# achiever04/face-recognition-platform

Hardware: AMD Instinct MI355X
Metric: faces/sec (detect+embed+match) on 1080p @ 100k gallery (higher is better)
Workload: dtype f16; 1 GPU; 32x1080x1920 BGR frames per GPU per step resident in HBM, host results out every step, 2 batches in flight per GPU (one handle = one stream each, used round-robin), forced K=10 faces/frame, 100000-identity fp16 gallery, FRPDet detector fp16 + ArcFace IResNet-100 fp16 (synthetic seeded weights); batch_frames=32, faces_per_frame=10, gallery=100000, streams=1, lanes=2, lane_warmup_steps=20

## Files before the change

face-recognition-platform_amd/csrc/aux_kernels.hip:

```cpp
#include <hip/hip_runtime.h>
#include <stdint.h>
#include "frp_internal.h"

namespace frp {

typedef _Float16 half8 __attribute__((ext_vector_type(8)));

__global__ __launch_bounds__(256) void preprocess_kernel(const uint8_t* __restrict__ src, int B, int H, int W,
                                                         long row_stride, long frame_stride,
                                                         _Float16* __restrict__ out, int Hc, int Wc, int rgb_in) {
    const long total = (long)B * Hc * Wc;
    for (long i = (long)blockIdx.x * blockDim.x + threadIdx.x; i < total; i += (long)gridDim.x * blockDim.x) {
        const int x = (int)(i % Wc);
        const long r = i / Wc;
        const int y = (int)(r % Hc);
        const int b = (int)(r / Hc);
        float c0 = 0.f, c1 = 0.f, c2 = 0.f;
        if (y < H && x < W) {
            const uint8_t* p = src + b * frame_stride + y * row_stride + 3L * x;
            c0 = (float)p[0]; c1 = (float)p[1]; c2 = (float)p[2];
        }
        const float r_ = rgb_in ? c0 : c2, g_ = c1, b_ = rgb_in ? c2 : c0;
        half8 v;
        v[0] = (_Float16)((r_ - 127.5f) * (1.0f / 128.0f));
// ... 11 lines not shown
    const int grid = (int)((total + 255) / 256 < 16384 ? (total + 255) / 256 : 16384);
    hipLaunchKernelGGL(preprocess_kernel, dim3(grid), dim3(256), 0, stream, bgr, B, H, W, row_stride, frame_stride,
                       out, Hc, Wc, rgb_in);
    return hipGetLastError();
}

__global__ __launch_bounds__(256) void compact_faces_kernel(const int32_t* __restrict__ counts, int B, int max_faces,
                                                            int32_t* __restrict__ face_slot, int32_t* __restrict__ n_faces) {
    __shared__ int offs[1024 + 1];
    if (threadIdx.x == 0) {
        int acc = 0;
        for (int b = 0; b < B; ++b) { offs[b] = acc; acc += counts[b]; }
        offs[B] = acc;
        *n_faces = acc;
    }
    __syncthreads();
    for (int b = threadIdx.x; b < B; b += blockDim.x) {
        const int c = counts[b], o = offs[b];
        for (int k = 0; k < c; ++k) face_slot[o + k] = b * max_faces + k;
    }
}

hipError_t launch_compact_faces(const int32_t* counts, int B, int max_faces, int32_t* face_slot, int32_t* n_faces,
                                hipStream_t stream) {
    if (B <= 0 || B > 1024) return hipErrorInvalidValue;
    hipLaunchKernelGGL(compact_faces_kernel, dim3(1), dim3(256), 0, stream, counts, B, max_faces, face_slot, n_faces);
    return hipGetLastError();
}

__constant__ float kTemplate[10] = {38.2946f, 51.6963f, 73.5318f, 51.5014f, 56.0252f, 71.7366f,
                                    41.5493f, 92.3655f, 70.7299f, 92.2041f};

#define ALIGN_SPLIT 7
__global__ __launch_bounds__(256) void align_kernel(AlignParams p) {
    const int f = blockIdx.x / ALIGN_SPLIT, part = blockIdx.x - f * ALIGN_SPLIT;
    if (f >= p.n_faces || (p.n_dev && f >= *p.n_dev)) return;
    const int slot = p.face_slot ? p.face_slot[f] : f;
    const int b = p.face_slot ? slot / p.max_faces : 0;
    const float* k = p.kps + (long)slot * 10;
    double msx = 0, msy = 0, mdx = 0, mdy = 0;
    for (int i = 0; i < 5; ++i) { msx += k[2 * i]; msy += k[2 * i + 1]; mdx += kTemplate[2 * i]; mdy += kTemplate[2 * i + 1]; }
    msx /= 5; msy /= 5; mdx /= 5; mdy /= 5;
    double num_a = 0, num_b = 0, den = 0;
    for (int i = 0; i < 5; ++i) {
        const double sx = k[2 * i] - msx, sy = k[2 * i + 1] - msy;
        const double dx = kTemplate[2 * i] - mdx, dy = kTemplate[2 * i + 1] - mdy;
        num_a += sx * dx + sy * dy;
        num_b += sx * dy - sy * dx;
        den += sx * sx + sy * sy;
    }
    const bool ok = den > 1e-12 && (num_a * num_a + num_b * num_b) > 1e-24;
    const double a = ok ? num_a / den : 1.0, bb = ok ? num_b / den : 0.0;
    const double tx = mdx - (a * msx - bb * msy), ty = mdy - (bb * msx + a * msy);
    const double det = a * a + bb * bb;
    const float i00 = (float)(a / det), i01 = (float)(bb / det), i10 = (float)(-bb / det), i11 = (float)(a / det);
    const float itx = (float)(-(a * tx + bb * ty) / det), ity = (float)(-(-bb * tx + a * ty) / det);
    const uint8_t* img = p.frames + (long)b * p.frame_stride;
    _Float16* out = p.chips + (long)f * (FRP_CHIP_PIX * 8);
    const int c_r = p.rgb_in ? 0 : 2, c_b = p.rgb_in ? 2 : 0;
    constexpr int kPart = FRP_CHIP_PIX / ALIGN_SPLIT;
    static_assert(kPart * ALIGN_SPLIT == FRP_CHIP_PIX, "chip rows must split evenly");
    for (int i = part * kPart + threadIdx.x; i < (part + 1) * kPart; i += blockDim.x) {
        const int v = i / 112, u = i - v * 112;
        const float sx = fminf(fmaxf(i00 * (float)u + i01 * (float)v + itx, -2.f), (float)(p.W + 1));
        const float sy = fminf(fmaxf(i10 * (float)u + i11 * (float)v + ity, -2.f), (float)(p.H + 1));
        const float fx0 = floorf(sx), fy0 = floorf(sy);
        const int x0 = (int)fx0, y0 = (int)fy0;
        const float ax = sx - fx0, ay = sy - fy0;
        unsigned char tap[4][3];
        float wgt[4];
        const int bx_max = 3 * p.W - 8;
        int bx = 3 * x0;
        bx = bx < 0 ? 0 : (bx > bx_max ? bx_max : bx);
#pragma unroll
        for (int dy = 0; dy < 2; ++dy) {
            const int yy = y0 + dy;
            const int yc = yy < 0 ? 0 : (yy >= p.H ? p.H - 1 : yy);
            unsigned long long v;
            __builtin_memcpy(&v, img + (long)yc * p.row_stride + bx, 8);
#pragma unroll
            for (int dx = 0; dx < 2; ++dx) {
                const int xx = x0 + dx;
                const bool inside = ok && (unsigned)xx < (unsigned)p.W && (unsigned)yy < (unsigned)p.H;
                int o = 3 * xx - bx;
                o = o < 0 ? 0 : (o > 5 ? 5 : o);
                const unsigned pix = (unsigned)(v >> (8 * o));
                tap[dy * 2 + dx][0] = (unsigned char)(pix >> (8 * c_r));
                tap[dy * 2 + dx][1] = (unsigned char)(pix >> 8);
                tap[dy * 2 + dx][2] = (unsigned char)(pix >> (8 * c_b));
                wgt[dy * 2 + dx] = inside ? (dx ? ax : 1.f - ax) * (dy ? ay : 1.f - ay) : 0.f;
            }
        }
        float acc[3] = {0.f, 0.f, 0.f};
#pragma unroll
        for (int k = 0; k < 4; ++k) {
            acc[0] += wgt[k] * (float)tap[k][0];
            acc[1] += wgt[k] * (float)tap[k][1];
            acc[2] += wgt[k] * (float)tap[k][2];
        }
        half8 o;
        o[0] = (_Float16)((acc[0] - 127.5f) * (1.0f / 127.5f));
        o[1] = (_Float16)((acc[1] - 127.5f) * (1.0f / 127.5f));
        o[2] = (_Float16)((acc[2] - 127.5f) * (1.0f / 127.5f));
        o[3] = o[4] = o[5] = o[6] = o[7] = (_Float16)0.f;
        *reinterpret_cast<half8*>(out + (long)i * 8) = o;
    }
}

hipError_t launch_align(const AlignParams& p, hipStream_t stream) {
    if (p.n_faces <= 0) return hipSuccess;
    if (!p.frames || !p.kps || !p.chips || p.H <= 0 || p.W < 3) return hipErrorInvalidValue;
    hipLaunchKernelGGL(align_kernel, dim3(p.n_faces * ALIGN_SPLIT), dim3(256), 0, stream, p);
    return hipGetLastError();
}

__global__ __launch_bounds__(256) void chips_to_blob_kernel(const uint8_t* __restrict__ chips, long total,
                                                            _Float16* __restrict__ out) {
    for (long i = (long)blockIdx.x * blockDim.x + threadIdx.x; i < total; i += (long)gridDim.x * blockDim.x) {
        const uint8_t* p = chips + 3 * i;
        half8 o;
        o[0] = (_Float16)(((float)p[2] - 127.5f) * (1.0f / 127.5f));
        o[1] = (_Float16)(((float)p[1] - 127.5f) * (1.0f / 127.5f));
        o[2] = (_Float16)(((float)p[0] - 127.5f) * (1.0f / 127.5f));
        o[3] = o[4] = o[5] = o[6] = o[7] = (_Float16)0.f;
        *reinterpret_cast<half8*>(out + i * 8) = o;
    }
}

hipError_t launch_chips_to_blob(const uint8_t* chips, int M, _Float16* out, hipStream_t stream) {
    if (M <= 0) return hipSuccess;
    const long total = (long)M * FRP_CHIP_PIX;
    const int grid = (int)((total + 255) / 256 < 8192 ? (total + 255) / 256 : 8192);
    hipLaunchKernelGGL(chips_to_blob_kernel, dim3(grid), dim3(256), 0, stream, chips, total, out);
    return hipGetLastError();
}

__device__ __forceinline__ float wave_sum(float v) {
#pragma unroll
    for (int o = 32; o > 0; o >>= 1) v += __shfl_xor(v, o);
    return v;
}

__global__ __launch_bounds__(256) void l2norm_kernel(float* __restrict__ emb, _Float16* __restrict__ emb16, int M, int D,
                                                      const float* __restrict__ partials, int ksplit, const float* __restrict__ bias,
                                                      const int32_t* __restrict__ n_dev, int fc_ktot, int n_cu) {
// ... 181 lines not shown
```

face-recognition-platform_amd/csrc/decode_nms.hip:

```cpp
#include <hip/hip_runtime.h>
#include <stdint.h>
#include "frp_internal.h"

namespace frp {

#define NMS_CAP 1024
#define NT 1024

__device__ __forceinline__ unsigned sortable16(unsigned short h) {
    if ((h & 0x7fffu) > 0x7c00u) return 0u;
    return (h & 0x8000u) ? (unsigned)(unsigned short)(~h) : (unsigned)(h | 0x8000u);
}
__device__ __forceinline__ bool is_candidate(_Float16 lg, float lt) {
    return lt == -INFINITY ? true : (float)lg >= lt;
}

struct FrameView {
    const _Float16 *h0, *h1, *h2;
    int w0, w1, w2;
    int e0, e1;
};

__device__ __forceinline__ const _Float16* anchor_ptr(const FrameView& fv, int idx, int& level, int& x, int& y) {
    level = idx < fv.e0 ? 0 : (idx < fv.e1 ? 1 : 2);
    const int li = idx - (level == 0 ? 0 : (level == 1 ? fv.e0 : fv.e1));
    const int wl = level == 0 ? fv.w0 : (level == 1 ? fv.w1 : fv.w2);
    const _Float16* base = level == 0 ? fv.h0 : (level == 1 ? fv.h1 : fv.h2);
    const int pos = li >> 1, a = li & 1;
    y = pos / wl;
    x = pos - y * wl;
    return base + (long)pos * 32 + a * 15;
}

__device__ __forceinline__ FrameView frame_view(const DecodeParams& p, int b, int& A) {
    FrameView fv;
    fv.h0 = p.head[0] + (long)b * p.hl[0] * p.wl[0] * 32;
    fv.h1 = p.head[1] + (long)b * p.hl[1] * p.wl[1] * 32;
    fv.h2 = p.head[2] + (long)b * p.hl[2] * p.wl[2] * 32;
    fv.w0 = p.wl[0]; fv.w1 = p.wl[1]; fv.w2 = p.wl[2];
    fv.e0 = p.hl[0] * p.wl[0] * 2;
    fv.e1 = fv.e0 + p.hl[1] * p.wl[1] * 2;
    A = fv.e1 + p.hl[2] * p.wl[2] * 2;
    return fv;
}

__global__ __launch_bounds__(256) void gather_logits_kernel(DecodeParams p) {
    int A;
    const FrameView fv = frame_view(p, blockIdx.y, A);
    const int i = blockIdx.x * 256 + threadIdx.x;
    if (i >= A) return;
    int lv, x, y;
    p.logits[(long)blockIdx.y * A + i] = anchor_ptr(fv, i, lv, x, y)[0];
}

__global__ __launch_bounds__(NT) void decode_nms_kernel(DecodeParams p) {
    __shared__ unsigned long long keys[NMS_CAP];
    __shared__ int hist[4096];
    __shared__ float bx1[NMS_CAP], by1[NMS_CAP], bx2[NMS_CAP], by2[NMS_CAP], barea[NMS_CAP];
    __shared__ unsigned char supp[NMS_CAP];
    __shared__ int s_cnt, s_digit, s_need, s_keepn;
    __shared__ int s_keep[FRP_MAX_FACES_CAP];
    __shared__ int wsum[NT / 64];

    const int b = blockIdx.x;
    const int tid = threadIdx.x;
    int A;
    const FrameView fv = frame_view(p, b, A);
    const float lt = p.logit_thresh;

    if (tid == 0) { s_cnt = 0; s_keepn = 0; }
    __syncthreads();
    const _Float16* dense = p.logits + (long)b * A;
    int local = 0;
    for (int i = tid; i < A; i += NT) local += is_candidate(dense[i], lt) ? 1 : 0;
#pragma unroll
    for (int o = 32; o > 0; o >>= 1) local += __shfl_xor(local, o);
    if ((tid & 63) == 0) atomicAdd(&s_cnt, local);
    __syncthreads();
    const int total = s_cnt;
    __syncthreads();

    unsigned long long T = 0ull;
    if (total > NMS_CAP) {
        unsigned long long prefix = 0ull;
        int need = NMS_CAP;
        for (int pass = 0; pass < 3; ++pass) {
            const int shift = 24 - 12 * pass;
            for (int i = tid; i < 4096; i += NT) hist[i] = 0;
            __syncthreads();
            for (int i = tid; i < A; i += NT) {
                const _Float16 lg = dense[i];
                if (is_candidate(lg, lt)) {
                    const unsigned long long k = ((unsigned long long)sortable16(__builtin_bit_cast(unsigned short, lg)) << 20) |
                                                 (unsigned long long)(0xFFFFF - i);
                    if (pass == 0 || (k >> (shift + 12)) == prefix) atomicAdd(&hist[(int)((k >> shift) & 0xFFF)], 1);
                }
            }
            __syncthreads();
            const int b0 = tid * 4;
            const int h0 = hist[b0], h1 = hist[b0 + 1], h2 = hist[b0 + 2], h3 = hist[b0 + 3];
            const int mine = h0 + h1 + h2 + h3;
            int v = mine;
#pragma unroll
            for (int o = 1; o < 64; o <<= 1) {
                const int n = __shfl_down(v, o);
                if ((tid & 63) + o < 64) v += n;
            }
            if ((tid & 63) == 0) wsum[tid >> 6] = v;
            __syncthreads();
            int above_waves = 0;
            for (int w = (tid >> 6) + 1; w < NT / 64; ++w) above_waves += wsum[w];
            const int suffix_incl = v + above_waves;
            const int above = suffix_incl - mine;
            int c = above;
            if (c < need && need <= c + h3) { s_digit = b0 + 3; s_need = need - c; }
            c += h3;
            if (c < need && need <= c + h2) { s_digit = b0 + 2; s_need = need - c; }
            c += h2;
            if (c < need && need <= c + h1) { s_digit = b0 + 1; s_need = need - c; }
            c += h1;
            if (c < need && need <= c + h0) { s_digit = b0; s_need = need - c; }
            __syncthreads();
            prefix = (prefix << 12) | (unsigned long long)s_digit;
            need = s_need;
            __syncthreads();
        }
        T = prefix;
    }

    if (tid == 0) s_cnt = 0;
    for (int i = tid; i < NMS_CAP; i += NT) { keys[i] = 0ull; supp[i] = 0; }
    __syncthreads();
    for (int i = tid; i < A; i += NT) {
        const _Float16 lg = dense[i];
        if (is_candidate(lg, lt)) {
            const unsigned long long k = ((unsigned long long)sortable16(__builtin_bit_cast(unsigned short, lg)) << 20) |
                                         (unsigned long long)(0xFFFFF - i);
            if (k >= T) {
                const int s = atomicAdd(&s_cnt, 1);
                if (s < NMS_CAP) keys[s] = k | (1ull << 40);
            }
        }
    }
    __syncthreads();
    const int n = s_cnt < NMS_CAP ? s_cnt : NMS_CAP;

    for (int k2 = 2; k2 <= NMS_CAP; k2 <<= 1) {
        for (int j = k2 >> 1; j > 0; j >>= 1) {
            const int i = tid;
            const int ixj = i ^ j;
            if (ixj > i) {
                const unsigned long long a = keys[i], c = keys[ixj];
                const bool desc = (i & k2) == 0;
                if (desc ? (a < c) : (a > c)) { keys[i] = c; keys[ixj] = a; }
            }
            __syncthreads();
        }
    }

    if (tid < n) {
        const int idx = 0xFFFFF - (int)(keys[tid] & 0xFFFFF);
        int lv, x, y;
        const _Float16* q = anchor_ptr(fv, idx, lv, x, y);
        const float s = (float)(8 << lv);
        const float cx = (float)(x * (8 << lv)), cy = (float)(y * (8 << lv));
        const float x1 = cx - (float)q[1] * s, y1 = cy - (float)q[2] * s;
        const float x2 = cx + (float)q[3] * s, y2 = cy + (float)q[4] * s;
        bx1[tid] = x1; by1[tid] = y1; bx2[tid] = x2; by2[tid] = y2;
        barea[tid] = (x2 - x1 + 1.0f) * (y2 - y1 + 1.0f);
    }
    __syncthreads();

    const int K = p.max_faces;
    for (int i = 0; i < n; ++i) {
        if (supp[i]) continue;
        if (tid == 0) s_keep[s_keepn] = i;
// ... 59 lines not shown
        const float fy = sy - (float)y0, fx = sx - (float)x0;
        const uint8_t* p00 = src + (((long)b * H + y0) * W + x0) * 3;
        const uint8_t* p01 = src + (((long)b * H + y0) * W + x1) * 3;
        const uint8_t* p10 = src + (((long)b * H + y1) * W + x0) * 3;
        const uint8_t* p11 = src + (((long)b * H + y1) * W + x1) * 3;
        uint8_t* o = dst + i * 3;
#pragma unroll
        for (int c = 0; c < 3; ++c) {
            const float top = (float)p00[c] * (1.0f - fx) + (float)p01[c] * fx;
            const float bot = (float)p10[c] * (1.0f - fx) + (float)p11[c] * fx;
            const float v = top * (1.0f - fy) + bot * fy;
            o[c] = (uint8_t)fminf(fmaxf(floorf(v + 0.5f), 0.0f), 255.0f);
        }
    }
}

hipError_t launch_resize_u8(const uint8_t* src, int B, int H, int W, uint8_t* dst, int Hs, int Ws, hipStream_t stream) {
    if (!src || !dst || B <= 0 || H <= 0 || W <= 0 || Hs <= 0 || Ws <= 0) return hipErrorInvalidValue;
    const long total = (long)B * Hs * Ws;
    const int grid = (int)((total + 255) / 256 < 16384 ? (total + 255) / 256 : 16384);
    hipLaunchKernelGGL(resize_u8_kernel, dim3(grid), dim3(256), 0, stream, src, B, H, W, dst, Hs, Ws,
                       (float)H / (float)Hs, (float)W / (float)Ws);
    return hipGetLastError();
}

hipError_t launch_decode_nms(const DecodeParams& p, hipStream_t stream) {
    if (p.B <= 0 || p.max_faces <= 0 || p.max_faces > FRP_MAX_FACES_CAP) return hipErrorInvalidValue;
    long A = 0;
    for (int l = 0; l < 3; ++l) {
        if (!p.head[l] || p.hl[l] <= 0 || p.wl[l] <= 0) return hipErrorInvalidValue;
        A += (long)p.hl[l] * p.wl[l] * 2;
    }
    if (A > 0xFFFFF) return hipErrorInvalidValue;
    if (!p.boxes || !p.kps || !p.scores || !p.counts || !p.logits) return hipErrorInvalidValue;
    hipLaunchKernelGGL(gather_logits_kernel, dim3((unsigned)((A + 255) / 256), p.B), dim3(256), 0, stream, p);
    hipError_t e = hipGetLastError();
    if (e != hipSuccess) return e;
    hipLaunchKernelGGL(decode_nms_kernel, dim3(p.B), dim3(NT), 0, stream, p);
    return hipGetLastError();
}

}
```

face-recognition-platform_amd/csrc/frp_api.cpp:

```cpp
#include <hip/hip_runtime.h>

#include <algorithm>
#include <cmath>
#include <cstdio>
#include <cstdlib>
#include <cstring>
#include <mutex>
#include <string>
#include <vector>

#include "frp.h"
#include "frp_blob.h"
#include "frp_internal.h"
#include "frp_handle.h"

using namespace frp;

#define FRP_WINO_MIN_FACES 128
Switches frp::read_switches() {
    auto set = [](const char* n) { return getenv(n) ? 1 : 0; };
    const char *sm = getenv("FRP_SMALL_M"), *wm = getenv("FRP_WINO_MIN_FACES");
    Switches s{};
    s.small_m = !sm ? 0 : (sm[0] == '0' ? -1 : 1);
    s.wino_min_faces = wm ? atoi(wm) : FRP_WINO_MIN_FACES;
// ... 49 lines not shown
    FRPCHK(ensure(h, h->anchor, s * 4));
    FRPCHK(ensure(h, h->counts, (size_t)B * 4));
    FRPCHK(ensure(h, h->face_slot, s * 4));
    FRPCHK(ensure(h, h->nfaces, 16));
    return FRP_OK;
}

struct DetOut {
    float *boxes, *kps, *scores;
    int32_t* counts;
};

int run_decode(frp_handle* h, const void* const head[3], const int dims[3][2], int B, int K, float det_thresh, float nms_iou, uint32_t flags,
               const DetOut* out = nullptr) {
    DecodeParams dp{};
    size_t anchors = 0;
    for (int l = 0; l < 3; ++l) {
        dp.head[l] = (const _Float16*)head[l];
        dp.hl[l] = dims[l][0];
        dp.wl[l] = dims[l][1];
        anchors += (size_t)dp.hl[l] * dp.wl[l] * 2;
    }
    dp.B = B;
    dp.max_faces = K;
    const bool forced = flags & FRP_FLAG_FORCED_K;
    dp.logit_thresh = forced ? -INFINITY : logit_threshold(det_thresh);
    dp.nms_iou = forced ? 2.0f : nms_iou;
    if (out) {
        dp.boxes = out->boxes; dp.kps = out->kps; dp.scores = out->scores; dp.counts = out->counts;
    } else {
        dp.boxes = (float*)h->boxes.p; dp.kps = (float*)h->kps.p; dp.scores = (float*)h->scores.p;
        dp.anchor = (int32_t*)h->anchor.p; dp.counts = (int32_t*)h->counts.p;
    }
    FRPCHK(ensure(h, h->dense_logits, (size_t)B * anchors * 2));
    dp.logits = (_Float16*)h->dense_logits.p;
    const hipError_t e = launch_decode_nms(dp, h->stream);
    if (e != hipSuccess) return fail(h, FRP_ERR_HIP, std::string("decode_nms: ") + hipGetErrorString(e));
    return FRP_OK;
}

int compact_faces(frp_handle* h, int B, int K) {
    hipError_t e = launch_compact_faces((const int32_t*)h->counts.p, B, K, (int32_t*)h->face_slot.p, (int32_t*)h->nfaces.p, h->stream);
    if (e != hipSuccess) return fail(h, FRP_ERR_HIP, std::string("compact_faces: ") + hipGetErrorString(e));
    return FRP_OK;
}

StemParams stem_params(const frp_handle* h, uint32_t flags) {
    StemParams sp{};
    sp.frames = h->det_scaled ? (const uint8_t*)h->scaled.p : (const uint8_t*)h->frames.p;
    sp.B = h->rB; sp.H = h->dH; sp.W = h->dW;
    sp.row_stride = (long)h->dW * 3; sp.frame_stride = (long)h->dH * h->dW * 3;
    sp.Hc = h->canvas_h; sp.Wc = h->canvas_w; sp.Ho = sp.Hc / 2; sp.Wo = sp.Wc / 2;
    sp.rgb_in = (flags & FRP_FLAG_RGB) ? 1 : 0;
    return sp;
}

bool det_wino(const frp_handle* h) {
    return (long)h->rB * (h->canvas_h / 8) * (h->canvas_w / 8) >= 2L * 240 * (h->n_cu > 0 ? h->n_cu : 256);
}

int run_detect(frp_handle* h, const Switches& sw, int K, float det_thresh, float nms_iou, uint32_t flags, const DetOut* out = nullptr) {
    if (!h->have_weights) return fail(h, FRP_ERR_NO_WEIGHTS, "no weights loaded");
    if (h->rB <= 0) return fail(h, FRP_ERR_INVALID, "no resident frames (call frp_upload_frames)");
    if (K <= 0 || K > FRP_MAX_FACES_CAP) return fail(h, FRP_ERR_INVALID, "max_faces out of range");
    const int B = h->rB, Hc = h->canvas_h, Wc = h->canvas_w;
    const bool fused = h->det.det_stem && !sw.no_fused_stem;
    FRPCHK(plan_net(h, h->det, B, Hc, Wc, fused));
    if (!out) FRPCHK(ensure_results(h, B, K));
// ... 330 lines not shown
    h->cfg.max_batch = 32; h->cfg.max_faces = 10; h->cfg.max_h = 1080; h->cfg.max_w = 1920; h->cfg.profile = 0;
    if (cfg) {
        if (cfg->struct_size != (int32_t)sizeof(frp_config)) { delete h; return FRP_ERR_INVALID; }
        if (cfg->max_batch > 0) h->cfg.max_batch = cfg->max_batch;
        if (cfg->max_faces > 0) h->cfg.max_faces = std::min<int>(cfg->max_faces, FRP_MAX_FACES_CAP);
        if (cfg->max_h > 0) h->cfg.max_h = cfg->max_h;
        if (cfg->max_w > 0) h->cfg.max_w = cfg->max_w;
        h->cfg.profile = cfg->profile ? 1 : 0;
    }
    bool ok = hipSetDevice(device) == hipSuccess && hipStreamCreateWithFlags(&h->stream, hipStreamNonBlocking) == hipSuccess;
    for (int i = 0; ok && i < EV_COUNT; ++i) ok = hipEventCreate(&h->ev[i]) == hipSuccess;
    ok = ok && hipHostMalloc((void**)&h->h_nfaces, 64, hipHostMallocDefault) == hipSuccess;
    if (ok) {
        hipDeviceProp_t prop;
        if (hipGetDeviceProperties(&prop, device) == hipSuccess && prop.multiProcessorCount > 0) h->n_cu = prop.multiProcessorCount;
    }
    ok = ok && init_ingest(h);
    if (!ok) { frp_destroy(h); return FRP_ERR_HIP; }
    h->ctr.struct_size = sizeof(frp_counters);
    *out = h;
    return FRP_OK;
}

void frp_destroy(frp_handle* h) {
    if (!h) return;
    (void)hipSetDevice(h->device);
    if (h->stream) (void)hipStreamSynchronize(h->stream);
    if (h->in.copy_stream) (void)hipStreamSynchronize(h->in.copy_stream);
    dist_shutdown(h);
    drop_graphs(h);
    for (DevBuf& b : h->det.bufs) release(b);
    for (DevBuf& b : h->emb.bufs) release(b);
    DevBuf* all[] = {&h->wdata, &h->frames, &h->boxes, &h->kps, &h->scores, &h->counts, &h->anchor, &h->face_slot, &h->nfaces,
                     &h->pyr_boxes, &h->pyr_kps, &h->pyr_scores, &h->pyr_counts, &h->m.q16, &h->m.part_cos, &h->m.part_idx, &h->m.best_cos, &h->m.best_idx, &h->m.hit_cnt, &h->m.hit_idx, &h->m.hit_cos, &h->m.q_groups, &h->m.frame_groups_dev, &h->g_groups_dev, &h->scratch, &h->splitk_ws, &h->dense_logits, &h->scaled, &h->gallery,
                     &h->g_reserved, &h->gx, &h->gx_q, &h->gx_out, &h->det_hashes, &h->quality_in, &h->quality_out,
                     &h->jenc_in, &h->jenc_coef, &h->jenc_work, &h->jenc_bits, &h->jenc_out, &h->enh_in, &h->enh_out};
    for (DevBuf* b : all) release(*b);
    for (int i = 0; i < EV_COUNT; ++i) if (h->ev[i]) (void)hipEventDestroy(h->ev[i]);
    if (h->m.frame_groups_ev) (void)hipEventDestroy(h->m.frame_groups_ev);
    release_tracks(h);
    if (h->h_nfaces) (void)hipHostFree(h->h_nfaces);
    if (h->pin_stage) (void)hipHostFree(h->pin_stage);
    release_ingest(h);
    if (h->stream) (void)hipStreamDestroy(h->stream);
    delete h;
}

const char* frp_last_error(const frp_handle* h) { return h ? h->err.c_str() : "null handle"; }

int frp_load_weights(frp_handle* h, const void* blob, size_t bytes) {
    if (!h) return FRP_ERR_INVALID;
    Guard g(h);
    h->have_weights = false;
    ++h->alloc_epoch;
    if (!blob || bytes < sizeof(frp_blob_header)) return fail(h, FRP_ERR_BLOB, "blob too small");
    frp_blob_header hd;
    memcpy(&hd, blob, sizeof(hd));
    if (memcmp(hd.magic, FRP_BLOB_MAGIC, 8) != 0 || hd.version != FRP_BLOB_VERSION || hd.header_bytes != sizeof(frp_blob_header))
        return fail(h, FRP_ERR_BLOB, "bad magic/version");
    if (hd.data_offset > bytes || hd.data_bytes > bytes - hd.data_offset) return fail(h, FRP_ERR_BLOB, "data section out of range");
    if (hd.emb_dim != FRP_EMB_DIM || hd.emb_size != FRP_CHIP || hd.det_in_ch != 8 || hd.emb_in_ch != 8 || hd.det_num_anchors != 2)
        return fail(h, FRP_ERR_BLOB, "unsupported network geometry");
    std::vector<unsigned char> image;
    FRPCHK(load_program(h, hd, (const unsigned char*)blob, bytes, read_switches(), image));
    FRPCHK(ensure(h, h->wdata, image.size()));
    HIPCHK(h, hipMemcpyAsync(h->wdata.p, image.data(), image.size(), hipMemcpyHostToDevice, h->stream));
    HIPCHK(h, hipStreamSynchronize(h->stream));
// ... 312 lines not shown
```

face-recognition-platform_amd/csrc/frp_handle.h:

```cpp
#pragma once
#include <hip/hip_runtime.h>

#include <algorithm>
#include <mutex>
#include <string>
#include <utility>
#include <vector>

#include "frp.h"
#include "frp_blob.h"
#include "frp_internal.h"
#include "net_program.h"

enum { EV_START = 0, EV_H2D, EV_PRE, EV_DET, EV_DEC, EV_ALIGN, EV_EMB, EV_L2, EV_MATCH, EV_D2H, EV_COUNT };

struct Ingest {
    frp::DevBuf frames_next;
    int nB = 0, nH = 0, nW = 0;
    bool next_valid = false;
    hipStream_t copy_stream = nullptr;
    hipEvent_t ev_next_ready = nullptr, ev_next_free = nullptr;
    std::vector<void*> pinned;
    void* jpeg_pin[2] = {nullptr, nullptr};
    size_t jpeg_pin_cap[2] = {0, 0};
// ... 52 lines not shown
    bool groups = false;
    bool tracked = false, track_matched = false;
    int pend_cap = 0;
    double pend_flops = 0.0, pend_f8flops = 0.0;
};

struct frp_handle {
    int device = 0;
    hipStream_t stream = nullptr;
    std::mutex mu;
    std::string err;
    frp_config cfg{};
    bool have_weights = false;
    frp_blob_header hdr{};
    frp::DevBuf wdata;
    frp::Net det, emb;
    frp::DevBuf frames;
    int rB = 0, rH = 0, rW = 0;
    int n_cu = 256;
    Ingest in;
    frp::DevBuf scaled;
    int dH = 0, dW = 0;
    bool det_scaled = false;
    int canvas_h = 0, canvas_w = 0;
    int det_op_limit = -1;
    std::vector<frp::NetGraph> graphs;
    std::vector<std::string> graph_seen, graph_bad;
    uint64_t alloc_epoch = 1;
    int64_t graph_replays = 0;
    void* comm = nullptr;
    int dist_rank = 0, dist_world = 0;
    frp::DevBuf det_hashes;
    bool det_hash_on = false;
    frp::DevBuf boxes, kps, scores, counts, anchor, face_slot, nfaces, scratch, splitk_ws, dense_logits;
    frp::DevBuf pyr_boxes, pyr_kps, pyr_scores, pyr_counts;
    Matcher m;
    Pass pass;
    Tracks trk;
    bool ev_pending = false;
    frp::DevBuf quality_in, quality_out;
    frp::DevBuf jenc_in, jenc_coef, jenc_work, jenc_bits, jenc_out;
    frp::DevBuf enh_in, enh_out;
    int32_t* h_nfaces = nullptr;
    unsigned char* pin_stage = nullptr;
    size_t pin_cap = 0;
    frp::DevBuf gallery;
    int64_t g_rows = 0;
    frp::DevBuf g_reserved;
    bool g_exact = false;
    frp::DevBuf gx, gx_q, gx_out;
    std::vector<uint32_t> g_groups;
    frp::DevBuf g_groups_dev;
    bool g_groups_dev_ok = false;
    hipEvent_t ev[EV_COUNT]{};
    frp_counters ctr{};
};

namespace frp {

inline int fail(frp_handle* h, int code, const std::string& msg) {
    if (h) h->err = msg;
    return code;
}

#define HIPCHK(h, expr)                                                                              \
    do {                                                                                             \
        hipError_t _e = (expr);                                                                      \
// ... 84 lines not shown
```

face-recognition-platform_amd/csrc/frp_internal.h:

```cpp
#pragma once
#include <hip/hip_runtime.h>
#include <stdint.h>
#include <type_traits>

#define FRP_ACT_NONE 0
#define FRP_ACT_RELU 1
#define FRP_ACT_PRELU 2
#define FRP_FLAG_BORDER_BIAS 1
#define FRP_FLAG_OUT_F32 2
#define FRP_FLAG_RES_UP2 4
#define FRP_FLAG_FLATTEN 8
#define FRP_FLAG_F8 32
#define FRP_FLAG_OUT_FP8 64
#define FRP_CHIP_PIX (112 * 112)
#ifndef FRP_MAX_FACES_CAP
#define FRP_MAX_FACES_CAP 128
#endif

#include "jpeg_host.h"
#include "jpeg_selfsync.h"

namespace frp {

struct Switches {
// ... 181 lines not shown
    const _Float16* w;
    const float* bias;
    _Float16* out;
};
hipError_t launch_stem_u8(const StemParams& p, hipStream_t stream);

struct Stem12Params {
    const uint8_t* frames;
    int B, H, W;
    long row_stride, frame_stride;
    int Hc, Wc;
    int Ho1, Wo1;
    int Ho2, Wo2;
    int rgb_in;
    const _Float16* w1;
    const float* bias1;
    const _Float16* w2;
    const float* bias2;
    _Float16* out;
};
hipError_t launch_stem12_u8(const Stem12Params& p, hipStream_t stream);

struct EmbStemParams {
    const _Float16* x;
    int M, H, W;
    const _Float16* w;
    const float* bias;
    const float* slope;
    _Float16* out;
    const int32_t* n_dev;
};
hipError_t launch_emb_stem(const EmbStemParams& p, hipStream_t stream);

struct DecodeParams {
    const _Float16* head[3];
    int hl[3], wl[3];
    int B, max_faces;
    float logit_thresh, nms_iou;
    float* boxes;
    float* kps;
    float* scores;
    int32_t* anchor;
    int32_t* counts;
    _Float16* logits;
};
hipError_t launch_decode_nms(const DecodeParams& p, hipStream_t stream);

#define FRP_PYRAMID_MAX_SCALES 4
#define FRP_PYRAMID_MAX_CAND 512
struct PyramidMergeParams {
    const float* boxes;
    const float* kps;
    const float* scores;
    const int32_t* counts;
    int S, B, P, max_faces;
    int frame_h, frame_w;
    int det_h[FRP_PYRAMID_MAX_SCALES], det_w[FRP_PYRAMID_MAX_SCALES];
    float nms_iou;
    float* out_boxes;
    float* out_kps;
    float* out_scores;
    int32_t* out_anchor;
    int32_t* out_counts;
    float rx[FRP_PYRAMID_MAX_SCALES], ry[FRP_PYRAMID_MAX_SCALES];
};
hipError_t launch_pyramid_merge(PyramidMergeParams p, hipStream_t stream);

struct JpegParams {
    const int16_t* coef;
    const uint16_t* qtab;
    uint8_t* planes;
    uint8_t* frames;
    int B, W, H, components;
    int bx[3], by[3];
    int blocks_per_image;
    long plane_off[3], plane_img;
    int hs, vs;
    int cw, ch;
// ... 271 lines not shown
```

Measured before the change: 28520 faces/s.

## Split decode top-k selection across slices and batch align tap loads

Decode no longer gathers dense logits and runs a per-frame radix select over every anchor in one block. A new multi-block kernel now selects the top candidates from each slice of anchors into a compact key buffer, and the NMS kernel then radix-selects only over those merged keys. Separately, the align kernel computes the similarity transform once per block in shared memory and issues all bilinear row loads before the arithmetic so that memory latency overlaps. The cost is an extra selection buffer and a second radix pass, plus higher register use in align.

New measurement: 28630 faces/s (median of 6 runs). No clear change (+0.4%).

```diff
diff --git a/face-recognition-platform_amd/csrc/aux_kernels.hip b/face-recognition-platform_amd/csrc/aux_kernels.hip
--- a/face-recognition-platform_amd/csrc/aux_kernels.hip
+++ b/face-recognition-platform_amd/csrc/aux_kernels.hip
@@ -67,63 +67,88 @@
                                     41.5493f, 92.3655f, 70.7299f, 92.2041f};
 
 #define ALIGN_SPLIT 7
-__global__ __launch_bounds__(256) void align_kernel(AlignParams p) {
+#define ALIGN_NT 256
+__global__ __launch_bounds__(ALIGN_NT) void align_kernel(AlignParams p) {
+    __shared__ float s_inv[6];
+    __shared__ int s_ok;
     const int f = blockIdx.x / ALIGN_SPLIT, part = blockIdx.x - f * ALIGN_SPLIT;
     if (f >= p.n_faces || (p.n_dev && f >= *p.n_dev)) return;
     const int slot = p.face_slot ? p.face_slot[f] : f;
     const int b = p.face_slot ? slot / p.max_faces : 0;
-    const float* k = p.kps + (long)slot * 10;
-    double msx = 0, msy = 0, mdx = 0, mdy = 0;
-    for (int i = 0; i < 5; ++i) { msx += k[2 * i]; msy += k[2 * i + 1]; mdx += kTemplate[2 * i]; mdy += kTemplate[2 * i + 1]; }
-    msx /= 5; msy /= 5; mdx /= 5; mdy /= 5;
-    double num_a = 0, num_b = 0, den = 0;
-    for (int i = 0; i < 5; ++i) {
-        const double sx = k[2 * i] - msx, sy = k[2 * i + 1] - msy;
-        const double dx = kTemplate[2 * i] - mdx, dy = kTemplate[2 * i + 1] - mdy;
-        num_a += sx * dx + sy * dy;
-        num_b += sx * dy - sy * dx;
-        den += sx * sx + sy * sy;
-    }
-    const bool ok = den > 1e-12 && (num_a * num_a + num_b * num_b) > 1e-24;
-    const double a = ok ? num_a / den : 1.0, bb = ok ? num_b / den : 0.0;
-    const double tx = mdx - (a * msx - bb * msy), ty = mdy - (bb * msx + a * msy);
-    const double det = a * a + bb * bb;
-    const float i00 = (float)(a / det), i01 = (float)(bb / det), i10 = (float)(-bb / det), i11 = (float)(a / det);
-    const float itx = (float)(-(a * tx + bb * ty) / det), ity = (float)(-(-bb * tx + a * ty) / det);
+    if (threadIdx.x == 0) {
+        const float* k = p.kps + (long)slot * 10;
+        double msx = 0, msy = 0, mdx = 0, mdy = 0;
+        for (int i = 0; i < 5; ++i) { msx += k[2 * i]; msy += k[2 * i + 1]; mdx += kTemplate[2 * i]; mdy += kTemplate[2 * i + 1]; }
+        msx /= 5; msy /= 5; mdx /= 5; mdy /= 5;
+        double num_a = 0, num_b = 0, den = 0;
+        for (int i = 0; i < 5; ++i) {
+            const double sx = k[2 * i] - msx, sy = k[2 * i + 1] - msy;
+            const double dx = kTemplate[2 * i] - mdx, dy = kTemplate[2 * i + 1] - mdy;
+            num_a += sx * dx + sy * dy;
+            num_b += sx * dy - sy * dx;
+            den += sx * sx + sy * sy;
+        }
+        const bool ok = den > 1e-12 && (num_a * num_a + num_b * num_b) > 1e-24;
+        const double a = ok ? num_a / den : 1.0, bb = ok ? num_b / den : 0.0;
+        const double tx = mdx - (a * msx - bb * msy), ty = mdy - (bb * msx + a * msy);
+        const double det = a * a + bb * bb;
+        s_inv[0] = (float)(a / det); s_inv[1] = (float)(bb / det); s_inv[2] = (float)(-bb / det); s_inv[3] = (float)(a / det);
+        s_inv[4] = (float)(-(a * tx + bb * ty) / det); s_inv[5] = (float)(-(-bb * tx + a * ty) / det);
+        s_ok = ok ? 1 : 0;
+    }
+    __syncthreads();
+    const float i00 = s_inv[0], i01 = s_inv[1], i10 = s_inv[2], i11 = s_inv[3], itx = s_inv[4], ity = s_inv[5];
+    const bool ok = s_ok != 0;
     const uint8_t* img = p.frames + (long)b * p.frame_stride;
     _Float16* out = p.chips + (long)f * (FRP_CHIP_PIX * 8);
     const int c_r = p.rgb_in ? 0 : 2, c_b = p.rgb_in ? 2 : 0;
     constexpr int kPart = FRP_CHIP_PIX / ALIGN_SPLIT;
     static_assert(kPart * ALIGN_SPLIT == FRP_CHIP_PIX, "chip rows must split evenly");
-    for (int i = part * kPart + threadIdx.x; i < (part + 1) * kPart; i += blockDim.x) {
+    constexpr int kPix = kPart / ALIGN_NT;
+    static_assert(kPix * ALIGN_NT == kPart, "every thread takes the same number of pixels");
+    float ax[kPix], ay[kPix];
+    int x0[kPix], y0[kPix], bx[kPix];
+    unsigned long long row[kPix][2];
+    const int bx_max = 3 * p.W - 8;
+#pragma unroll
+    for (int j = 0; j < kPix; ++j) {
+        const int i = part * kPart + j * ALIGN_NT + threadIdx.x;
         const int v = i / 112, u = i - v * 112;
         const float sx = fminf(fmaxf(i00 * (float)u + i01 * (float)v + itx, -2.f), (float)(p.W + 1));
         const float sy = fminf(fmaxf(i10 * (float)u + i11 * (float)v + ity, -2.f), (float)(p.H + 1));
         const float fx0 = floorf(sx), fy0 = floorf(sy);
-        const int x0 = (int)fx0, y0 = (int)fy0;
-        const float ax = sx - fx0, ay = sy - fy0;
+        x0[j] = (int)fx0; y0[j] = (int)fy0;
+        ax[j] = sx - fx0; ay[j] = sy - fy0;
+        int o = 3 * x0[j];
+        bx[j] = o < 0 ? 0 : (o > bx_max ? bx_max : o);
+#pragma unroll
+        for (int dy = 0; dy < 2; ++dy) {
+            const int yy = y0[j] + dy;
+            const int yc = yy < 0 ? 0 : (yy >= p.H ? p.H - 1 : yy);
+            __builtin_memcpy(&row[j][dy], img + (long)yc * p.row_stride + bx[j], 8);
+        }
+    }
+    __builtin_amdgcn_sched_barrier(0);
+#pragma unroll
+    for (int j = 0; j < kPix; ++j) {
+        const int i = part * kPart + j * ALIGN_NT + threadIdx.x;
         unsigned char tap[4][3];
         float wgt[4];
-        const int bx_max = 3 * p.W - 8;
-        int bx = 3 * x0;
-        bx = bx < 0 ? 0 : (bx > bx_max ? bx_max : bx);
 #pragma unroll
         for (int dy = 0; dy < 2; ++dy) {
-            const int yy = y0 + dy;
-            const int yc = yy < 0 ? 0 : (yy >= p.H ? p.H - 1 : yy);
-            unsigned long long v;
-            __builtin_memcpy(&v, img + (long)yc * p.row_stride + bx, 8);
+            const int yy = y0[j] + dy;
+            const unsigned long long v = row[j][dy];
 #pragma unroll
             for (int dx = 0; dx < 2; ++dx) {
-                const int xx = x0 + dx;
+                const int xx = x0[j] + dx;
                 const bool inside = ok && (unsigned)xx < (unsigned)p.W && (unsigned)yy < (unsigned)p.H;
-                int o = 3 * xx - bx;
+                int o = 3 * xx - bx[j];
                 o = o < 0 ? 0 : (o > 5 ? 5 : o);
                 const unsigned pix = (unsigned)(v >> (8 * o));
                 tap[dy * 2 + dx][0] = (unsigned char)(pix >> (8 * c_r));
                 tap[dy * 2 + dx][1] = (unsigned char)(pix >> 8);
                 tap[dy * 2 + dx][2] = (unsigned char)(pix >> (8 * c_b));
-                wgt[dy * 2 + dx] = inside ? (dx ? ax : 1.f - ax) * (dy ? ay : 1.f - ay) : 0.f;
+                wgt[dy * 2 + dx] = inside ? (dx ? ax[j] : 1.f - ax[j]) * (dy ? ay[j] : 1.f - ay[j]) : 0.f;
             }
         }
         float acc[3] = {0.f, 0.f, 0.f};
@@ -145,7 +170,7 @@
 hipError_t launch_align(const AlignParams& p, hipStream_t stream) {
     if (p.n_faces <= 0) return hipSuccess;
     if (!p.frames || !p.kps || !p.chips || p.H <= 0 || p.W < 3) return hipErrorInvalidValue;
-    hipLaunchKernelGGL(align_kernel, dim3(p.n_faces * ALIGN_SPLIT), dim3(256), 0, stream, p);
+    hipLaunchKernelGGL(align_kernel, dim3(p.n_faces * ALIGN_SPLIT), dim3(ALIGN_NT), 0, stream, p);
     return hipGetLastError();
 }
 
diff --git a/face-recognition-platform_amd/csrc/decode_nms.hip b/face-recognition-platform_amd/csrc/decode_nms.hip
--- a/face-recognition-platform_amd/csrc/decode_nms.hip
+++ b/face-recognition-platform_amd/csrc/decode_nms.hip
@@ -4,7 +4,7 @@
 
 namespace frp {
 
-#define NMS_CAP 1024
+#define NMS_CAP FRP_NMS_CAP
 #define NT 1024
 
 __device__ __forceinline__ unsigned sortable16(unsigned short h) {
@@ -13,6 +13,9 @@
 }
 __device__ __forceinline__ bool is_candidate(_Float16 lg, float lt) {
     return lt == -INFINITY ? true : (float)lg >= lt;
+}
+__device__ __forceinline__ unsigned long long anchor_key(unsigned short lg_bits, int anchor) {
+    return ((unsigned long long)sortable16(lg_bits) << 20) | (unsigned long long)(0xFFFFF - anchor);
 }
 
 struct FrameView {
@@ -30,6 +33,12 @@
     y = pos / wl;
     x = pos - y * wl;
     return base + (long)pos * 32 + a * 15;
+}
+__device__ __forceinline__ const _Float16* logit_ptr(const FrameView& fv, int idx) {
+    const int level = idx < fv.e0 ? 0 : (idx < fv.e1 ? 1 : 2);
+    const int li = idx - (level == 0 ? 0 : (level == 1 ? fv.e0 : fv.e1));
+    const _Float16* base = level == 0 ? fv.h0 : (level == 1 ? fv.h1 : fv.h2);
+    return base + (long)(li >> 1) * 32 + (li & 1) * 15;
 }
 
 __device__ __forceinline__ FrameView frame_view(const DecodeParams& p, int b, int& A) {
@@ -44,13 +53,99 @@
     return fv;
 }
 
-__global__ __launch_bounds__(256) void gather_logits_kernel(DecodeParams p) {
+template <class Each>
+__device__ __forceinline__ unsigned long long radix_select(Each each, int need, int* hist, int* wsum, int* s_digit, int* s_need) {
+    const int tid = threadIdx.x;
+    unsigned long long prefix = 0ull;
+    for (int pass = 0; pass < 3; ++pass) {
+        const int shift = 24 - 12 * pass;
+        for (int i = tid; i < 4096; i += NT) hist[i] = 0;
+        __syncthreads();
+        each([&](unsigned long long k) {
+            if (pass == 0 || (k >> (shift + 12)) == prefix) atomicAdd(&hist[(int)((k >> shift) & 0xFFF)], 1);
+        });
+        __syncthreads();
+        const int b0 = tid * 4;
+        const int h0 = hist[b0], h1 = hist[b0 + 1], h2 = hist[b0 + 2], h3 = hist[b0 + 3];
+        const int mine = h0 + h1 + h2 + h3;
+        int v = mine;
+#pragma unroll
+        for (int o = 1; o < 64; o <<= 1) {
+            const int n = __shfl_down(v, o);
+            if ((tid & 63) + o < 64) v += n;
+        }
+        if ((tid & 63) == 0) wsum[tid >> 6] = v;
+        __syncthreads();
+        int above_waves = 0;
+        for (int w = (tid >> 6) + 1; w < NT / 64; ++w) above_waves += wsum[w];
+        const int suffix_incl = v + above_waves;
+        const int above = suffix_incl - mine;
+        int c = above;
+        if (c < need && need <= c + h3) { *s_digit = b0 + 3; *s_need = need - c; }
+        c += h3;
+        if (c < need && need <= c + h2) { *s_digit = b0 + 2; *s_need = need - c; }
+        c += h2;
+        if (c < need && need <= c + h1) { *s_digit = b0 + 1; *s_need = need - c; }
+        c += h1;
+        if (c < need && need <= c + h0) { *s_digit = b0; *s_need = need - c; }
+        __syncthreads();
+        prefix = (prefix << 12) | (unsigned long long)*s_digit;
+        need = *s_need;
+        __syncthreads();
+    }
+    return prefix;
+}
+
+__global__ __launch_bounds__(NT) void decode_select_kernel(DecodeParams p) {
+    __shared__ unsigned short lg[FRP_DECODE_SLICE_MAX];
+    __shared__ int hist[4096];
+    __shared__ int s_cnt, s_digit, s_need;
+    __shared__ int wsum[NT / 64];
+
+    const int s = blockIdx.x, b = blockIdx.y;
+    const int tid = threadIdx.x;
     int A;
-    const FrameView fv = frame_view(p, blockIdx.y, A);
-    const int i = blockIdx.x * 256 + threadIdx.x;
-    if (i >= A) return;
-    int lv, x, y;
-    p.logits[(long)blockIdx.y * A + i] = anchor_ptr(fv, i, lv, x, y)[0];
+    const FrameView fv = frame_view(p, b, A);
+    const float lt = p.logit_thresh;
+    const int a0 = s * p.L;
+    const int n_own = A - a0 < p.L ? A - a0 : p.L;
+
+    if (tid == 0) s_cnt = 0;
+    __syncthreads();
+    int local = 0;
+#pragma unroll 4
+    for (int i = tid; i < n_own; i += NT) {
+        const _Float16 v = logit_ptr(fv, a0 + i)[0];
+        lg[i] = __builtin_bit_cast(unsigned short, v);
+        local += is_candidate(v, lt) ? 1 : 0;
+    }
+#pragma unroll
+    for (int o = 32; o > 0; o >>= 1) local += __shfl_xor(local, o);
+    if ((tid & 63) == 0) atomicAdd(&s_cnt, local);
+    __syncthreads();
+    const int total = s_cnt;
+    __syncthreads();
+
+    auto each = [&](auto f) {
+        for (int i = tid; i < n_own; i += NT) {
+            const unsigned short h = lg[i];
+            if (is_candidate(__builtin_bit_cast(_Float16, h), lt)) f(anchor_key(h, a0 + i));
+        }
+    };
+    unsigned long long T = 0ull;
+    if (total > NMS_CAP) T = radix_select(each, NMS_CAP, hist, wsum, &s_digit, &s_need);
+
+    if (tid == 0) s_cnt = 0;
+    __syncthreads();
+    unsigned long long* dst = p.sel_keys + ((long)b * p.S + s) * NMS_CAP;
+    each([&](unsigned long long k) {
+        if (k >= T) {
+            const int slot = atomicAdd(&s_cnt, 1);
+            if (slot < NMS_CAP) dst[slot] = k;
+        }
+    });
+    __syncthreads();
+    if (tid == 0) p.sel_cnt[b * p.S + s] = s_cnt < NMS_CAP ? s_cnt : NMS_CAP;
 }
 
 __global__ __launch_bounds__(NT) void decode_nms_kernel(DecodeParams p) {
@@ -66,82 +161,28 @@
     const int tid = threadIdx.x;
     int A;
     const FrameView fv = frame_view(p, b, A);
-    const float lt = p.logit_thresh;
+
+    const unsigned long long* sk = p.sel_keys + (long)b * p.S * NMS_CAP;
+    const int32_t* sc = p.sel_cnt + b * p.S;
+    int total = 0;
+    for (int s = 0; s < p.S; ++s) total += sc[s];
+    auto each = [&](auto f) {
+        for (int s = 0; s < p.S; ++s)
+            if (tid < sc[s]) f(sk[(long)s * NMS_CAP + tid]);
+    };
+
+    unsigned long long T = 0ull;
+    if (total > NMS_CAP) T = radix_select(each, NMS_CAP, hist, wsum, &s_digit, &s_need);
 
     if (tid == 0) { s_cnt = 0; s_keepn = 0; }
-    __syncthreads();
-    const _Float16* dense = p.logits + (long)b * A;
-    int local = 0;
-    for (int i = tid; i < A; i += NT) local += is_candidate(dense[i], lt) ? 1 : 0;
-#pragma unroll
-    for (int o = 32; o > 0; o >>= 1) local += __shfl_xor(local, o);
-    if ((tid & 63) == 0) atomicAdd(&s_cnt, local);
-    __syncthreads();
-    const int total = s_cnt;
-    __syncthreads();
-
-    unsigned long long T = 0ull;
-    if (total > NMS_CAP) {
-        unsigned long long prefix = 0ull;
-        int need = NMS_CAP;
-        for (int pass = 0; pass < 3; ++pass) {
-            const int shift = 24 - 12 * pass;
-            for (int i = tid; i < 4096; i += NT) hist[i] = 0;
-            __syncthreads();
-            for (int i = tid; i < A; i += NT) {
-                const _Float16 lg = dense[i];
-                if (is_candidate(lg, lt)) {
-                    const unsigned long long k = ((unsigned long long)sortable16(__builtin_bit_cast(unsigned short, lg)) << 20) |
-                                                 (unsigned long long)(0xFFFFF - i);
-                    if (pass == 0 || (k >> (shift + 12)) == prefix) atomicAdd(&hist[(int)((k >> shift) & 0xFFF)], 1);
-                }
-            }
-            __syncthreads();
-            const int b0 = tid * 4;
-            const int h0 = hist[b0], h1 = hist[b0 + 1], h2 = hist[b0 + 2], h3 = hist[b0 + 3];
-            const int mine = h0 + h1 + h2 + h3;
-            int v = mine;
-#pragma unroll
-            for (int o = 1; o < 64; o <<= 1) {
-                const int n = __shfl_down(v, o);
-                if ((tid & 63) + o < 64) v += n;
-            }
-            if ((tid & 63) == 0) wsum[tid >> 6] = v;
-            __syncthreads();
-            int above_waves = 0;
-            for (int w = (tid >> 6) + 1; w < NT / 64; ++w) above_waves += wsum[w];
-            const int suffix_incl = v + above_waves;
-            const int above = suffix_incl - mine;
-            int c = above;
-            if (c < need && need <= c + h3) { s_digit = b0 + 3; s_need = need - c; }
-            c += h3;
-            if (c < need && need <= c + h2) { s_digit = b0 + 2; s_need = need - c; }
-            c += h2;
-            if (c < need && need <= c + h1) { s_digit = b0 + 1; s_need = need - c; }
-            c += h1;
-            if (c < need && need <= c + h0) { s_digit = b0; s_need = need - c; }
-            __syncthreads();
-            prefix = (prefix << 12) | (unsigned long long)s_digit;
-            need = s_need;
-            __syncthreads();
-        }
-        T = prefix;
-    }
-
-    if (tid == 0) s_cnt = 0;
     for (int i = tid; i < NMS_CAP; i += NT) { keys[i] = 0ull; supp[i] = 0; }
     __syncthreads();
-    for (int i = tid; i < A; i += NT) {
-        const _Float16 lg = dense[i];
-        if (is_candidate(lg, lt)) {
-            const unsigned long long k = ((unsigned long long)sortable16(__builtin_bit_cast(unsigned short, lg)) << 20) |
-                                         (unsigned long long)(0xFFFFF - i);
-            if (k >= T) {
-                const int s = atomicAdd(&s_cnt, 1);
-                if (s < NMS_CAP) keys[s] = k | (1ull << 40);
-            }
-        }
-    }
+    each([&](unsigned long long k) {
+        if (k >= T) {
+            const int s = atomicAdd(&s_cnt, 1);
+            if (s < NMS_CAP) keys[s] = k | (1ull << 40);
+        }
+    });
     __syncthreads();
     const int n = s_cnt < NMS_CAP ? s_cnt : NMS_CAP;
 
@@ -267,11 +308,15 @@
         A += (long)p.hl[l] * p.wl[l] * 2;
     }
     if (A > 0xFFFFF) return hipErrorInvalidValue;
-    if (!p.boxes || !p.kps || !p.scores || !p.counts || !p.logits) return hipErrorInvalidValue;
-    hipLaunchKernelGGL(gather_logits_kernel, dim3((unsigned)((A + 255) / 256), p.B), dim3(256), 0, stream, p);
+    if (!p.boxes || !p.kps || !p.scores || !p.counts || !p.sel_keys || !p.sel_cnt) return hipErrorInvalidValue;
+    DecodeParams q = p;
+    const DecodeSlicePlan plan = decode_slice_plan(A, p.B);
+    q.S = plan.S; q.L = plan.L;
+    if (q.L > FRP_DECODE_SLICE_MAX || (long)q.S * q.L < A) return hipErrorInvalidValue;
+    hipLaunchKernelGGL(decode_select_kernel, dim3(q.S, q.B), dim3(NT), 0, stream, q);
     hipError_t e = hipGetLastError();
     if (e != hipSuccess) return e;
-    hipLaunchKernelGGL(decode_nms_kernel, dim3(p.B), dim3(NT), 0, stream, p);
+    hipLaunchKernelGGL(decode_nms_kernel, dim3(q.B), dim3(NT), 0, stream, q);
     return hipGetLastError();
 }
 
diff --git a/face-recognition-platform_amd/csrc/frp_api.cpp b/face-recognition-platform_amd/csrc/frp_api.cpp
--- a/face-recognition-platform_amd/csrc/frp_api.cpp
+++ b/face-recognition-platform_amd/csrc/frp_api.cpp
@@ -105,8 +105,9 @@
         dp.boxes = (float*)h->boxes.p; dp.kps = (float*)h->kps.p; dp.scores = (float*)h->scores.p;
         dp.anchor = (int32_t*)h->anchor.p; dp.counts = (int32_t*)h->counts.p;
     }
-    FRPCHK(ensure(h, h->dense_logits, (size_t)B * anchors * 2));
-    dp.logits = (_Float16*)h->dense_logits.p;
+    FRPCHK(ensure(h, h->decode_sel, decode_select_bytes((long)anchors, B)));
+    dp.sel_keys = (unsigned long long*)h->decode_sel.p;
+    dp.sel_cnt = (int32_t*)(dp.sel_keys + (size_t)B * decode_slice_plan((long)anchors, B).S * FRP_NMS_CAP);
     const hipError_t e = launch_decode_nms(dp, h->stream);
     if (e != hipSuccess) return fail(h, FRP_ERR_HIP, std::string("decode_nms: ") + hipGetErrorString(e));
     return FRP_OK;
@@ -503,7 +504,7 @@
     for (DevBuf& b : h->det.bufs) release(b);
     for (DevBuf& b : h->emb.bufs) release(b);
     DevBuf* all[] = {&h->wdata, &h->frames, &h->boxes, &h->kps, &h->scores, &h->counts, &h->anchor, &h->face_slot, &h->nfaces,
-                     &h->pyr_boxes, &h->pyr_kps, &h->pyr_scores, &h->pyr_counts, &h->m.q16, &h->m.part_cos, &h->m.part_idx, &h->m.best_cos, &h->m.best_idx, &h->m.hit_cnt, &h->m.hit_idx, &h->m.hit_cos, &h->m.q_groups, &h->m.frame_groups_dev, &h->g_groups_dev, &h->scratch, &h->splitk_ws, &h->dense_logits, &h->scaled, &h->gallery,
+                     &h->pyr_boxes, &h->pyr_kps, &h->pyr_scores, &h->pyr_counts, &h->m.q16, &h->m.part_cos, &h->m.part_idx, &h->m.best_cos, &h->m.best_idx, &h->m.hit_cnt, &h->m.hit_idx, &h->m.hit_cos, &h->m.q_groups, &h->m.frame_groups_dev, &h->g_groups_dev, &h->scratch, &h->splitk_ws, &h->decode_sel, &h->scaled, &h->gallery,
                      &h->g_reserved, &h->gx, &h->gx_q, &h->gx_out, &h->det_hashes, &h->quality_in, &h->quality_out,
                      &h->jenc_in, &h->jenc_coef, &h->jenc_work, &h->jenc_bits, &h->jenc_out, &h->enh_in, &h->enh_out};
     for (DevBuf* b : all) release(*b);
diff --git a/face-recognition-platform_amd/csrc/frp_handle.h b/face-recognition-platform_amd/csrc/frp_handle.h
--- a/face-recognition-platform_amd/csrc/frp_handle.h
+++ b/face-recognition-platform_amd/csrc/frp_handle.h
@@ -108,7 +108,7 @@
     int dist_rank = 0, dist_world = 0;
     frp::DevBuf det_hashes;
     bool det_hash_on = false;
-    frp::DevBuf boxes, kps, scores, counts, anchor, face_slot, nfaces, scratch, splitk_ws, dense_logits;
+    frp::DevBuf boxes, kps, scores, counts, anchor, face_slot, nfaces, scratch, splitk_ws, decode_sel;
     frp::DevBuf pyr_boxes, pyr_kps, pyr_scores, pyr_counts;
     Matcher m;
     Pass pass;
diff --git a/face-recognition-platform_amd/csrc/frp_internal.h b/face-recognition-platform_amd/csrc/frp_internal.h
--- a/face-recognition-platform_amd/csrc/frp_internal.h
+++ b/face-recognition-platform_amd/csrc/frp_internal.h
@@ -237,6 +237,16 @@
 };
 hipError_t launch_emb_stem(const EmbStemParams& p, hipStream_t stream);
 
+#define FRP_NMS_CAP 1024
+#define FRP_DECODE_SLICE_MAX 12288
+struct DecodeSlicePlan { int S, L; };
+inline DecodeSlicePlan decode_slice_plan(long A, int B) {
+    (void)B;
+    long L = (((A + 7) / 8) + 7) & ~7L;
+    L = L < FRP_NMS_CAP ? FRP_NMS_CAP : (L > FRP_DECODE_SLICE_MAX ? FRP_DECODE_SLICE_MAX : L);
+    const long S = A > L ? (A + L - 1) / L : 1;
+    return DecodeSlicePlan{(int)S, (int)L};
+}
 struct DecodeParams {
     const _Float16* head[3];
     int hl[3], wl[3];
@@ -247,8 +257,13 @@
     float* scores;
     int32_t* anchor;
     int32_t* counts;
-    _Float16* logits;
-};
+    unsigned long long* sel_keys;
+    int32_t* sel_cnt;
+    int S, L;
+};
+inline size_t decode_select_bytes(long A, int B) {
+    return (size_t)B * decode_slice_plan(A, B).S * (FRP_NMS_CAP * 8 + 4);
+}
 hipError_t launch_decode_nms(const DecodeParams& p, hipStream_t stream);
 
 #define FRP_PYRAMID_MAX_SCALES 4
```
